# thawro/pytorch-human-pose

Hardware: AMD Instinct MI355X
Metric: images/sec (fwd+decode) HigherHRNet-W32 512px (higher is better)
Workload: dtype bf16; 1 GPU; HigherHRNet-W32 inference bf16, batch 32 @ 512x512 per GPU (conv fwd on N(0,1) images + AE decode on constructed maps, 10 people/image, det_thr 0.05, tag_thr 0.5, adjust+refine); global_batch=32, parallelism=image-sharded replicas x1, no data-path collective

## Files before the change

### include/hhrnet.h

```cpp
#ifndef HHRNET_H
#define HHRNET_H
#include <stdint.h>

#ifdef __cplusplus
extern "C" {
#endif

#define HH_ABI_VERSION 3
#define HH_DTYPE_BF16 1
#define HH_DTYPE_FP8 2
#define HH_DTYPE_F16 3

typedef struct hh_net hh_net;
typedef struct hh_decoder hh_decoder;

int hh_abi_version(void);
const char *hh_last_error(void);

hh_net *hh_create(int num_kpts, int C, int dtype);
void hh_destroy(hh_net *net);

hh_net *hh_create_classifier(int C, int num_classes, int dtype);
int hh_forward_classifier(hh_net *net, const float *images, int B, int H, int W, float *logits, void *stream);

int hh_num_params(const hh_net *net);
const char *hh_param_name(const hh_net *net, int index);
int hh_param_shape(const hh_net *net, int index, int64_t shape[4]);

int hh_load_weights(hh_net *net, const char *name, const float *host, const int64_t *shape, int ndim);
int hh_finalize(hh_net *net);

int hh_calibrate(hh_net *net, const float *images, int B, int H, int W, int rounds, void *stream);

int hh_e4m3_encode(const float *x, int64_t n, unsigned char *out);
int hh_e4m3_decode(const unsigned char *x, int64_t n, float *out);

int hh_reserve(hh_net *net, int B, int H, int W);
int64_t hh_workspace_bytes(const hh_net *net);

int hh_forward(hh_net *net, const float *images, int B, int H, int W, float *init_heatmaps, float *deconv_heatmaps,
               int use_graph, void *stream);

int hh_set_multi_lane(hh_net *net, int enable);

int hh_debug_check_plan(const hh_net *net);

double hh_forward_flops(const hh_net *net, int B, int H, int W);

int hh_profile_enable(hh_net *net, int enable);
int hh_profile_count(const hh_net *net);
int hh_profile_get(hh_net *net, int index, int *cfg, double *flops, double *bytes, float *ms, float *kernel_ms, const char **layer);
int hh_profile_clock(hh_net *net, int index, double *ghz);
int hh_conv_config(int cfg, int out[7]);
int hh_conv_config_double_buffered(int cfg);

int hh_debug_conv_bench(int cfg, int B, int Hin, int Win, int cin, int cout, int with_res, int relu, int iters,
                        float *ms_per_launch, unsigned long long *stamps16, int ref_cfg, float *max_diff);

int hh_debug_bb_bench(int B, int H, int W, int iters, float *ms_per_launch, unsigned long long *stamps64);
int hh_debug_bb_compare(int B, int H, int W, int iters, float *max_diff, float *ms_classic, float *ms_pc);

int hh_debug_bb_cover(int B, int H, int W, int tall, int num_cus, int64_t counts[4]);

int hh_debug_stem_fused(hh_net *net, const float *images, int B, int H, int W, void *out16, void *stream);

int hh_set_taps(hh_net *net, int enable);
int hh_num_taps(const hh_net *net);
const char *hh_tap_name(const hh_net *net, int index);
int hh_tap_shape(const hh_net *net, int index, int64_t shape[4]);
int hh_tap_read(hh_net *net, int index, float *host_nchw);

int hh_preprocess_u8(const unsigned char *image_hwc, int h, int w, const double dst_to_src[6], float *out_nchw, int H, int W,
                     const float mean[3], const float stdv[3], void *stream);

typedef struct hh_image_desc {
    long long offset;
    int h, w;
    double dst_to_src[6];
} hh_image_desc;
int hh_preprocess_u8_batch(const unsigned char *images_base, const hh_image_desc *descs_dev, int n, float *out_nchw, int H, int W,
                           const float mean[3], const float stdv[3], void *stream);

int hh_flip_images(const float *images, float *out, int B, int C, int H, int W, void *stream);
int hh_flip_merge(float *hm, int64_t hm_bstride, const float *hm_flipped, int64_t hmf_bstride, const float *tags_flipped,
                  int64_t tf_bstride, float *tags_out, int64_t to_bstride, const int32_t *perm_host, int B, int K,
                  int h, int w, void *stream);

hh_decoder *hh_decoder_create(int num_kpts, int max_people, double det_thr, double tag_thr);
void hh_decoder_destroy(hh_decoder *dec);
int hh_decoder_reserve(hh_decoder *dec, int B, int H, int W, int E);
int hh_decoder_set_exact_topk(hh_decoder *dec, int enable);

#define HH_DECODE_FALLBACK 1
#define HH_DECODE_SOLVER_GUARD 2
int hh_decode(hh_decoder *dec, const float *hm_q, int64_t hm_q_bstride, const float *hm_h, int64_t hm_h_bstride,
              const float *const *tags_q, const int64_t *tags_bstride, int E, int B, int hq, int wq, int adjust,
              int refine, float *joints, float *scores, int32_t *num_people, int32_t *flags, void *stream);

int hh_parse(hh_decoder *dec, const float *hm_full, const float *tags_full, int E, int B, int H, int W, int adjust,
             int refine, float *joints, float *scores, int32_t *num_people, int32_t *flags, void *stream);

int hh_loss_heatmaps(const float *pred, int64_t pred_bstride, const float *target, const float *mask, int B, int K, int h, int w,
                     float *loss, float *grad, int64_t grad_bstride, double *scratch, void *stream);
int hh_loss_ae_grouping(const float *tags, int64_t tags_bstride, const int32_t *joints, const int32_t *num_people, int B, int P, int K,
                        int h, int w, float *push_pull, float *grad, int64_t grad_bstride, float push_scale, float pull_scale,
                        double *scratch, void *stream);

#define HH_TRAIN_MAX_STAGES 4
typedef struct hh_train_desc {
    long long image_offset, mask_offset;
// ... 440 lines not shown
```

### pytorch-human-pose_amd/csrc/capi.cpp

```cpp
#include <algorithm>
#include <cmath>
#include <cstdint>
#include <cstring>
#include <string>
#include <vector>

#include "../../include/hhrnet.h"
#include "engine.h"
#include "optim_math.h"
#include "grad_stats_math.h"
#include "ema_math.h"
#include "render_math.h"
#include "text_math.h"
#include "seg_overlay_math.h"
#include "panel_math.h"
#include "coco_eval_math.h"
#include "pose_score_math.h"
#include "cls_score_math.h"
#include "crowd_mask_math.h"
#include "track_math.h"
#include "jpeg_math.h"
#include "jpeg_dec_math.h"

const char *hh_get_error();
int hh_tap_read_impl(hh_net *n, int index, float *host);

template <class Frame>
static int draw_check_frames(const char *fn, const hh_render_desc *descs_host, int n, const char *call_why, bool no_table, int th, int tw, int *max_tiles,
                             Frame frame)
{
    if (n <= 0 || n > 65535) { hh_set_error(std::string(fn) + ": need 0 < n <= 65535"); return 1; }
    if (call_why) { hh_set_error(std::string(fn) + ": " + call_why); return 1; }
    int tiles = 1;
    for (int b = 0; b < n; ++b) {
        const hh_render_desc &d = descs_host[b];
        if (d.prim_count > 0 && no_table) { hh_set_error(std::string(fn) + ": null primitive table"); return 1; }
        const char *why = frame(d);
        if (why) { hh_set_error(std::string(fn) + ": frame " + std::to_string(b) + ": " + why); return 1; }
        tiles = std::max(tiles, ((d.h + th - 1) / th) * ((d.w + tw - 1) / tw));
    }
    if (max_tiles) *max_tiles = tiles;
    return 0;
}

extern "C" {

int hh_abi_version(void) { return HH_ABI_VERSION; }
const char *hh_last_error(void) { return hh_get_error(); }

static bool f16_switch_refused(hh_net *n)
{
    if (n->dtype != HH_DTYPE_F16 || (!n->sw.no_stem_fused && !n->sw.bb32_tile)) return false;
    hh_set_error(std::string("hh_create: HH_DTYPE_F16 with ") + (n->sw.no_stem_fused ? "HH_NO_STEM_FUSED" : "HH_BB32=tile") +
                 ": that debug switch reaches a kernel that has no fp16 form");
    delete n;
    return true;
}

hh_net *hh_create(int num_kpts, int C, int dtype)
{
    if (dtype != HH_DTYPE_BF16 && dtype != HH_DTYPE_FP8 && dtype != HH_DTYPE_F16) {
// ... 2133 lines not shown
    double A[6][6] = {}, b[6];
    for (int i = 0; i < 3; ++i) {
        A[2 * i][0] = A[2 * i + 1][3] = from[i][0];
        A[2 * i][1] = A[2 * i + 1][4] = from[i][1];
        A[2 * i][2] = A[2 * i + 1][5] = 1;
        b[2 * i] = to[i][0];
        b[2 * i + 1] = to[i][1];
    }
    if (lu_solve6(A, b)) { hh_set_error("hh_get_affine_transform: degenerate point set (scale_w or dst_w is 0)"); return 1; }
    for (int i = 0; i < 6; ++i) out[i] = b[i];
    return 0;
}

int hh_invert_affine(const double m[6], double out[6])
{
#pragma clang fp contract(off)
    double M[6];
    for (int i = 0; i < 6; ++i) M[i] = m[i];
    double D = M[0] * M[4] - M[1] * M[3];
    D = D != 0 ? 1. / D : 0;
    const double A11 = M[4] * D, A22 = M[0] * D;
    M[0] = A11; M[1] *= -D;
    M[3] *= -D; M[4] = A22;
    const double b1 = -M[0] * M[2] - M[1] * M[5];
    const double b2 = -M[3] * M[2] - M[4] * M[5];
    M[2] = b1; M[5] = b2;
    for (int i = 0; i < 6; ++i) out[i] = M[i];
    return 0;
}

int hh_warp_affine_u8(const unsigned char *image_hwc, int h, int w, const double dst_to_src[6], unsigned char *out_hwc, int H, int W, void *stream)
{
    if (!image_hwc || !out_hwc || h <= 0 || w <= 0 || H <= 0 || W <= 0) { hh_set_error("hh_warp_affine_u8: bad argument"); return 1; }
    HH_CHECK_HIP(launch_warp_affine_u8(image_hwc, h, w, dst_to_src, out_hwc, H, W, (hipStream_t)stream));
    return 0;
}

int hh_transform_coords(const float *xy_in, int n, double cx, double cy, double scale_w, double dst_w, double dst_h,
                        double *xy_out)
{
#pragma clang fp contract(off)
    double M[6];
    if (hh_get_affine_transform(cx, cy, scale_w, dst_w, dst_h, 1, M)) return 1;
    for (int i = 0; i < n; ++i) {
        const double x = (double)xy_in[2 * i + 0], y = (double)xy_in[2 * i + 1];
        xy_out[2 * i + 0] = M[0] * x + M[1] * y + M[2] * 1.0;
        xy_out[2 * i + 1] = M[3] * x + M[4] * y + M[5] * 1.0;
    }
    return 0;
}

}

extern "C" int hh_debug_conv_bench(int cfg, int B, int Hin, int Win, int cin, int cout, int with_res, int relu, int iters,
                                   float *ms_per_launch, unsigned long long *stamps16, int ref_cfg, float *max_diff)
{
    HH_CHECK_HIP(conv_init());
    if (cfg < 0 || cfg >= conv_num_configs()) { hh_set_error("bad cfg"); return 1; }
    ConvConfig c = conv_config(cfg);
    if (cin % c.KC) { hh_set_error("cin must be a multiple of the config's KC"); return 1; }
    const int coutp = (cout + c.cout_t() - 1) / c.cout_t() * c.cout_t();
    const int Ho = c.S == 2 ? Hin / 2 : Hin, Wo = c.S == 2 ? Win / 2 : Win;
    const size_t n_in = (size_t)B * Hin * Win * cin, n_out = (size_t)B * Ho * Wo * coutp;
    std::vector<bf16_raw> h_in(n_in), h_res(n_out);
    std::vector<float> W((size_t)cout * cin * c.KS * c.KS), scale(coutp, 1.f);
    uint32_t s = 12345u;
    auto rnd = [&]() { s = s * 1664525u + 1013904223u; return (bf16_raw)(0x3c00u + ((s >> 16) & 0x1ffu) + ((s >> 30) << 15)); };
    auto rndf = [&]() { s = s * 1664525u + 1013904223u; return ((int)(s >> 20) - 2048) / 16384.0f; };
    for (auto &v : h_in) v = rnd();
    for (auto &v : h_res) v = rnd();
    for (auto &v : W) v = rndf();
    bf16_raw *d_in, *d_out, *d_out2, *d_res, *d_zero;
    float *d_bias;
    HH_CHECK_HIP(hipMalloc((void **)&d_in, n_in * 2));
    HH_CHECK_HIP(hipMalloc((void **)&d_out, n_out * 2));
    HH_CHECK_HIP(hipMalloc((void **)&d_out2, n_out * 2));
    HH_CHECK_HIP(hipMalloc((void **)&d_res, n_out * 2));
    HH_CHECK_HIP(hipMalloc((void **)&d_bias, (size_t)coutp * 4));
    HH_CHECK_HIP(hipMalloc((void **)&d_zero, 256));
    HH_CHECK_HIP(hipMemcpy(d_in, h_in.data(), n_in * 2, hipMemcpyHostToDevice));
    HH_CHECK_HIP(hipMemcpy(d_res, h_res.data(), n_out * 2, hipMemcpyHostToDevice));
    HH_CHECK_HIP(hipMemset(d_bias, 0, (size_t)coutp * 4));
    HH_CHECK_HIP(hipMemset(d_zero, 0, 256));
    HH_CHECK_HIP(hipMemset(d_out, 0, n_out * 2));
    HH_CHECK_HIP(hipMemset(d_out2, 0, n_out * 2));
    unsigned long long *d_st = nullptr;
    HH_CHECK_HIP(hipMalloc((void **)&d_st, 16 * 8));
    HH_CHECK_HIP(hipMemset(d_st, 0, 16 * 8));
    hipStream_t st;
    HH_CHECK_HIP(hipStreamCreate(&st));
    auto run = [&](int k, bf16_raw *out, int n, float *ms_out) -> int {
        const ConvConfig cc = conv_config(k);
        std::vector<bf16_raw> packed;
        hh_pack_weights(W.data(), scale.data(), cc.KS, cin, cout, cc.KC, cc.cout_t(), false, 0, 0, packed);
        bf16_raw *d_w;
        HH_CHECK_HIP(hipMalloc((void **)&d_w, packed.size() * 2));
        HH_CHECK_HIP(hipMemcpy(d_w, packed.data(), packed.size() * 2, hipMemcpyHostToDevice));
        ConvParams p{};
        p.in = d_in; p.in_cs = cin; p.Hin = Hin; p.Win = Win; p.w = d_w; p.bias = d_bias;
        p.res = with_res ? d_res : nullptr; p.res_cs = coutp;
        p.out = out; p.out_cs = coutp; p.Hob = Ho; p.Wob = Wo; p.osy = p.osx = 1;
        p.Ho = Ho; p.Wo = Wo; p.cin = cin; p.cout_real = cout; p.cout_store = coutp; p.relu = relu;
        p.pad_y = p.pad_x = (cc.KS - 1) / 2; p.B = B; p.stamps = d_st;
        p.tiles_x = (Wo + cc.TW - 1) / cc.TW; p.tiles_y = (Ho + cc.th() - 1) / cc.th(); p.ncg = coutp / cc.cout_t();
        auto launch = [&]() { return conv_launch(k, p, st); };
        hipEvent_t e0, e1;
        HH_CHECK_HIP(hipEventCreate(&e0));
        HH_CHECK_HIP(hipEventCreate(&e1));
        for (int i = 0; i < 3; ++i) HH_CHECK_HIP(launch());
        HH_CHECK_HIP(hipEventRecord(e0, st));
        for (int i = 0; i < n; ++i) HH_CHECK_HIP(launch());
        HH_CHECK_HIP(hipEventRecord(e1, st));
        HH_CHECK_HIP(hipEventSynchronize(e1));
        float ms = 0;
        HH_CHECK_HIP(hipEventElapsedTime(&ms, e0, e1));
        if (ms_out) *ms_out = ms / n;
        hipEventDestroy(e0); hipEventDestroy(e1); hipFree(d_w);
        return 0;
    };
    if (run(cfg, d_out, iters, ms_per_launch)) return 1;
    if (stamps16) HH_CHECK_HIP(hipMemcpy(stamps16, d_st, 16 * 8, hipMemcpyDeviceToHost));
    if (max_diff) {
        if (run(ref_cfg, d_out2, 1, nullptr)) return 1;
        std::vector<bf16_raw> a(n_out), b2(n_out);
        HH_CHECK_HIP(hipMemcpy(a.data(), d_out, n_out * 2, hipMemcpyDeviceToHost));
        HH_CHECK_HIP(hipMemcpy(b2.data(), d_out2, n_out * 2, hipMemcpyDeviceToHost));
        float md = 0.f;
        for (size_t i = 0; i < n_out; ++i) {
            uint32_t ua = (uint32_t)a[i] << 16, ub = (uint32_t)b2[i] << 16;
            float fa, fb;
            memcpy(&fa, &ua, 4); memcpy(&fb, &ub, 4);
            const float d = fa > fb ? fa - fb : fb - fa;
            if (d > md || d != d) md = d;
        }
        *max_diff = md;
    }
    hipStreamDestroy(st);
    hipFree(d_in); hipFree(d_out); hipFree(d_out2); hipFree(d_res); hipFree(d_bias); hipFree(d_st); hipFree(d_zero);
    return 0;
}

extern "C" int hh_debug_bb_cover(int B, int H, int W, int tall, int num_cus, int64_t counts[4])
{
    long long c[4];
    if (!counts) { hh_set_error("hh_debug_bb_cover: counts is NULL"); return 1; }
    if (!bbpc_cover(B, H, W, tall, num_cus, c)) { hh_set_error("hh_debug_bb_cover: the launcher does not take this shape"); return 1; }
    for (int i = 0; i < 4; ++i) counts[i] = c[i];
    return 0;
}

extern "C" int hh_debug_bb_compare(int B, int H, int W, int iters, float *max_diff, float *ms_classic, float *ms_pc)
{
    HH_CHECK_HIP(conv_init());
    HH_CHECK_HIP(bb_fused_init());
    HH_CHECK_HIP(bbpc_init());
    const size_t n = (size_t)B * H * W * 32;
    std::vector<bf16_raw> h_in(n), h_w(2 * 9 * 32 * 32), h_o1(n), h_o2(n);
    std::vector<float> h_b(64);
    uint32_t s = 4242u;
    auto rnd = [&]() { s = s * 1664525u + 1013904223u; return (bf16_raw)(0x3c00u + ((s >> 16) & 0x1ffu) + ((s >> 30) << 15)); };
    for (auto &v : h_in) v = (bf16_raw)(rnd() + 0x0300u);
    for (auto &v : h_w) v = rnd();
    for (auto &v : h_b) { s = s * 1664525u + 1013904223u; v = ((int)(s >> 20) - 2048) * 1e-4f; }
    bf16_raw *d_in, *d_o1, *d_o2, *d_w;
    float *d_b;
    HH_CHECK_HIP(hipMalloc((void **)&d_in, n * 2));
    HH_CHECK_HIP(hipMalloc((void **)&d_o1, n * 2));
    HH_CHECK_HIP(hipMalloc((void **)&d_o2, n * 2));
    HH_CHECK_HIP(hipMalloc((void **)&d_w, h_w.size() * 2));
    HH_CHECK_HIP(hipMalloc((void **)&d_b, 64 * 4));
    HH_CHECK_HIP(hipMemcpy(d_in, h_in.data(), n * 2, hipMemcpyHostToDevice));
    HH_CHECK_HIP(hipMemcpy(d_w, h_w.data(), h_w.size() * 2, hipMemcpyHostToDevice));
    HH_CHECK_HIP(hipMemcpy(d_b, h_b.data(), 64 * 4, hipMemcpyHostToDevice));
    HH_CHECK_HIP(hipMemset(d_o1, 0xff, n * 2));
    HH_CHECK_HIP(hipMemset(d_o2, 0xff, n * 2));
    BBParams p{};
    p.in = d_in; p.in_cs = 32; p.out_cs = 32; p.w1 = d_w; p.w2 = d_w + 9 * 32 * 32; p.b1 = d_b; p.b2 = d_b + 32;
    p.B = B; p.H = H; p.W = W;
    unsigned long long *d_st = nullptr;
    HH_CHECK_HIP(hipMalloc((void **)&d_st, 72 * 8));
    HH_CHECK_HIP(hipMemset(d_st, 0, 72 * 8));
    p.stamps = d_st;
    int dev = 0;
    hipDeviceProp_t prop;
    HH_CHECK_HIP(hipGetDevice(&dev));
    HH_CHECK_HIP(hipGetDeviceProperties(&prop, dev));
    hipStream_t st;
    HH_CHECK_HIP(hipStreamCreate(&st));
    hipEvent_t e0, e1;
    HH_CHECK_HIP(hipEventCreate(&e0));
    HH_CHECK_HIP(hipEventCreate(&e1));
// ... 95 lines not shown
```

### pytorch-human-pose_amd/csrc/engine.cpp

```cpp
#include "engine.h"
#include "f16_host.h"

#include <cmath>
#include <cstdlib>
#include <cstring>

static thread_local std::string g_err;
LaunchProbe &hh_launch_probe()
{
    static thread_local LaunchProbe p;
    return p;
}
void hh_set_error(const std::string &msg) { g_err = msg; }
const char *hh_get_error() { return g_err.c_str(); }

PlanSwitches PlanSwitches::from_env()
{
    auto on = [](const char *name) { const char *v = getenv(name); return v && *v && strcmp(v, "0"); };
    auto is = [](const char *name, const char *val) { const char *v = getenv(name); return v && !strcmp(v, val); };
    PlanSwitches s;
    s.bb32_tile = is("HH_BB32", "tile");
    s.no_bb64 = on("HH_NO_BB64");
    s.no_stem_fused = on("HH_NO_STEM_FUSED");
    s.no_junc_pair = on("HH_NO_JUNC_PAIR");
    s.full_join = on("HH_FULL_JOIN");
    s.no_fusion_merge = on("HH_NO_FUSION_MERGE");
    s.no_fused_upsum = on("HH_NO_FUSED_UPSUM");
    s.poison_ws = on("HH_POISON_WS");
    s.poison_lds = on("HH_POISON_LDS");
    s.no_head_fold = on("HH_NO_HEAD_FOLD");
    s.no_trans_dual = on("HH_NO_TRANS_DUAL");
    s.no_conv_db = on("HH_NO_CONV_DB");
    s.no_final_fuse = on("HH_NO_FINAL_FUSE");
    s.keep_waits = on("HH_KEEP_WAITS");
    s.event_system_fence = on("HH_EVENT_SYSTEM_FENCE");
    s.bb_tall = on("HH_NO_BB_TALL") ? 0 : is("HH_BB_TALL", "always") ? 2 : 1;
    s.fp8_trunk8 = is("HH_FP8_TRUNK", "e4m3");
    s.fp8_heads8 = is("HH_FP8_HEADS", "e4m3");
    return s;
}

static inline int round_up(int v, int m) { return (v + m - 1) / m * m; }

static inline bf16_raw f2bf(float f)
{
    uint32_t u;
    memcpy(&u, &f, 4);
    if ((u & 0x7fffffffu) > 0x7f800000u) return (bf16_raw)((u >> 16) | 0x40);
    u += 0x7fffu + ((u >> 16) & 1u);
    return (bf16_raw)(u >> 16);
}
static inline float bf2f(bf16_raw h)
{
    uint32_t u = (uint32_t)h << 16;
    float f;
    memcpy(&f, &u, 4);
    return f;
}
bf16_raw hh_net::cvt16(float f) const { return act() ? hh_f32_to_f16(f) : f2bf(f); }
float hh_net::widen16(bf16_raw v) const { return act() ? hh_f16_to_f32(v) : bf2f(v); }
int hh_net::check_packed(const std::vector<bf16_raw> &packed, const std::string &param_name) const
{
    if (!act()) return 0;
    for (bf16_raw v : packed)
        if (hh_f16_is_inf(v)) {
            hh_set_error("hh_finalize: " + param_name + ": a BatchNorm-folded weight exceeds the fp16 range (+-65504); use a bf16 handle for this checkpoint");
            return 1;
        }
    return 0;
}

int hh_net::add_param(const std::string &name, std::vector<int64_t> shape, bool counter)
{
    ParamSlot p;
    p.name = name;
    p.shape = std::move(shape);
    p.counter = counter;
    param_index[name] = (int)params.size();
    params.push_back(std::move(p));
    return (int)params.size() - 1;
}

namespace {
struct Builder {
// ... 506 lines not shown
                        for (int j = 0; j < 8; ++j, ++o) {
                            const int co = cg * COUT_T + ci_o, ci = ch * KC + c8 * 8 + j;
                            if (co >= cout || ci >= cin) continue;
                            float v;
                            if (transposed) v = W[(((size_t)ci * cout + co) * 4 + ky) * 4 + kx];
                            else v = W[(((size_t)co * cin + ci) * ks + ky) * ks + kx];
                            packed[o] = act_dtype ? hh_f32_to_f16(v * scale[co]) : f2bf(v * scale[co]);
                        }
            }
}

int hh_family_pick(int ks, int stride, int cin_pad, int coutp, int *KC, int *NT)
{
    if (ks == 3 && stride == 1) *KC = (cin_pad % 32 == 0) ? 32 : 16;
    else if (ks == 1) *KC = (cin_pad % 32 == 0) ? 32 : 16;
    else *KC = 16;
    *NT = (coutp % 64 == 0) ? 2 : 1;
    for (int i = 0; i < conv_num_configs(); ++i) {
        const ConvConfig &c = conv_config(i);
        if (c.KS == ks && c.S == stride && c.KC == *KC && c.NT == *NT && !c.DB) return 0;
    }
    return 1;
}

float hh_net::bn_fold(const std::string &bn, int co, const float *cb, float *shift) const
{
    const float g = param(bn + ".weight")[co], bta = param(bn + ".bias")[co];
    const float mu = param(bn + ".running_mean")[co], var = param(bn + ".running_var")[co];
    const float sc = g / std::sqrt(var + 1e-5f);
    *shift = cb ? bta + (*cb - mu) * sc : bta - mu * sc;
    return sc;
}

void hh_net::fold_layer(const ConvLayer &l, int coutp, std::vector<float> &scale, std::vector<float> &shift) const
{
    scale.assign(coutp, 0.f);
    shift.assign(coutp, 0.f);
    for (int co = 0; co < l.cout; ++co) {
        const float cb = l.bias.empty() ? 0.f : param(l.bias)[co];
        if (l.bn.empty()) { scale[co] = 1.f; shift[co] = cb; }
        else scale[co] = bn_fold(l.bn, co, &cb, &shift[co]);
    }
}

int hh_net::finalize()
{
    for (auto &p : params)
        if (!p.loaded && !p.counter) { hh_set_error("hh_finalize: parameter never loaded: " + p.name); return 1; }
    HH_CHECK_HIP(conv_init());
    HH_CHECK_HIP(bb_fused_init());
    HH_CHECK_HIP(stem_fused_init());
    HH_CHECK_HIP(bbpc_init());
    HH_CHECK_HIP(bb64_fused_init());
    HH_CHECK_HIP(junction_init());
    if (dtype == 2 && kind != 0) { hh_set_error("hh_finalize: the fp8 path covers HigherHRNet only"); return 1; }
    {
        int dev = 0;
        hipDeviceProp_t prop;
        HH_CHECK_HIP(hipGetDevice(&dev));
        HH_CHECK_HIP(hipGetDeviceProperties(&prop, dev));
        num_cus = prop.multiProcessorCount;
    }
    for (auto &l : layers) {
        if (l.stem) {
            const std::vector<float> &W = param(l.conv + ".weight");
            std::vector<bf16_raw> packed(64 * 32, 0);
            std::vector<float> shift(64);
            for (int co = 0; co < 64; ++co) {
                const float sc = bn_fold(l.bn, co, nullptr, &shift[co]);
                for (int t = 0; t < 27; ++t) {
                    const int kk = t / 16, hh = (t % 16) / 8, j = t % 8;
                    packed[((((co / 32) * 2 + kk) * 2 + hh) * 32 + co % 32) * 8 + j] = cvt16(W[(size_t)co * 27 + t] * sc);
                }
            }
            if (check_packed(packed, l.conv + ".weight")) return 1;
            if (hh_upload(&l.d_w, packed.data(), packed.size() * 2) || hh_upload(&l.d_bias, shift.data(), 64 * 4)) return 1;
            continue;
        }
        if (dtype == 2 && !l.hi) continue;
        const int cin_pad0 = round_up(l.cin, 16), coutp = round_up(l.cout, 32);
        if (l.stem2) { l.KC = 64; l.NT = 2; }
        else if (hh_family_pick(l.ks, l.stride, cin_pad0, coutp, &l.KC, &l.NT)) {
            hh_set_error("no kernel family for conv " + l.conv);
            return 1;
        }
        l.db = !sw.no_conv_db && !l.stem2 && l.ks == 3 && l.stride == 1 && !l.transposed && l.mconv.empty() && l.cin >= 128 &&
               l.cin % 16 == 0 && coutp % 64 == 0;
        if (l.db) { l.KC = 16; l.NT = 2; }
        l.cin_pad = round_up(l.cin, l.KC);
        const int COUT_T = 32 * l.NT;
        l.ncg = coutp / COUT_T;
        if (!l.mconv.empty()) {
            std::vector<float> Wm((size_t)l.cout * l.cin * 9, 0.f), one(coutp, 1.f), shift(coutp, 0.f);
            int c0 = 0;
            for (size_t m = 0; m < l.mconv.size(); ++m) {
                if (l.mcin[m] % l.KC) { hh_set_error("merged fusion conv: input width not a multiple of the chunk size"); return 1; }
                const std::vector<float> &Wj = param(l.mconv[m] + ".weight");
                for (int co = 0; co < l.cout; ++co) {
                    float sh;
                    const float sc = bn_fold(l.mbn[m], co, nullptr, &sh);
                    shift[co] += sh;
                    for (int ci = 0; ci < l.mcin[m]; ++ci)
                        for (int t = 0; t < 9; ++t) Wm[((size_t)co * l.cin + c0 + ci) * 9 + t] = Wj[((size_t)co * l.mcin[m] + ci) * 9 + t] * sc;
                    if (act())
                        for (int i = 0; i < l.mcin[m] * 9; ++i)
                            if (hh_f16_is_inf(hh_f32_to_f16(Wj[(size_t)co * l.mcin[m] * 9 + i] * sc))) return check_packed({0x7c00}, l.mconv[m] + ".weight");
// ... 418 lines not shown
    else if (act()) { hh_set_error("hh_forward: the tile-form 32-channel block (tensors of 2 GB and more) has no fp16 form"); return 1; }
    else HH_CHECK_HIP(bb_fused_launch(p, num_cus, s));
    return 0;
}

int hh_net::enqueue_conv(const Op &op, int B, int H, int W, float *o1, float *o2, hipStream_t s)
{
    const ConvLayer &l = layers[op.layer];
    const TensorDesc &ti = tensors[op.in];
    ConvParams p{};
    hh_conv_geometry(p, l, op, B, H >> ti.shift, W >> ti.shift, o1, o2);
    p.in = dtype == 2 ? ti.ptr16 : ti.ptr; p.in_cs = ti.C; p.in_coff = op.in_coff;
    p.w = l.d_w; p.bias = l.d_bias;
    if (op.out >= 0) {
        const TensorDesc &to = tensors[op.out];
        p.out = dtype == 2 ? to.ptr16 : to.ptr; p.out_cs = to.C; p.out_coff = op.out_coff;
    }
    if (op.res >= 0) {
        const TensorDesc &tr = tensors[op.res];
        p.res = dtype == 2 ? tr.ptr16 : tr.ptr; p.res_cs = tr.C; p.res_coff = op.res_coff;
    }
    if (op.in2 >= 0) {
        const TensorDesc &t2 = tensors[op.in2];
        if (t2.C != ti.C || t2.shift != ti.shift || (op.in3 >= 0 && (tensors[op.in3].C != ti.C || tensors[op.in3].shift != ti.shift))) {
            hh_set_error("merged fusion conv: inputs differ in shape or pixel stride");
            return 1;
        }
        p.nch0 = l.mcin[0] / l.KC;
        p.nch1 = l.mcin[1] / l.KC;
        p.src_delta1 = t2.ptr - (ti.ptr + op.in_coff);
        if (op.in3 >= 0) p.src_delta2 = tensors[op.in3].ptr - (ti.ptr + op.in_coff);
    }
    p.cout_store = op.cout_store >= 0 ? op.cout_store : round_up(l.cout, 8);
    if (op.layer2 >= 0) {
        const ConvLayer &l2 = layers[op.layer2];
        const TensorDesc &t2 = tensors[op.out2];
        const ConvConfig &c = conv_config(0);
        if (dtype == 2 || l.ks != 3 || l.stride != 1 || l.KC != c.KC || l.NT != c.NT || l.db || l.ncg != 1 || l2.ks != 3 || l2.stride != 2 || l2.KC != 16 ||
            l2.NT != 2 || l2.ncg != 1 || l2.cin_pad != l.cin_pad || t2.shift != ti.shift + 1) {
            hh_set_error("plan: the dual transition launch does not fit conv_mfma.hip (HH_NO_TRANS_DUAL=1)");
            return 1;
        }
        p.w2 = l2.d_w; p.bias2 = l2.d_bias;
        p.out2 = t2.ptr; p.out2_cs = t2.C; p.out2_coff = 0;
        p.Ho2 = p.Hin / 2; p.Wo2 = p.Win / 2;
        p.tiles_x = (p.Wo + c.TW - 1) / c.TW;
        p.tiles_y = (p.Ho + c.th() - 1) / c.th();
        if (prof_enabled && prof_record(op, HH_CFG_TRANS_DUAL, op_cost(op, B, H, W), &p.clk)) return 1;
        HH_CHECK_HIP(conv_dual_launch(p, s, act()));
        return 0;
    }
    const int cfg = hh_pick_config(l.ks, l.stride, l.KC, l.NT, p.Wo, l.db);
    const ConvConfig &c = conv_config(cfg);
    p.tiles_x = (p.Wo + c.TW - 1) / c.TW;
    p.tiles_y = (p.Ho + c.th() - 1) / c.th();
    if (prof_enabled && prof_record(op, cfg, op_cost(op, B, H, W), &p.clk)) return 1;
    HH_CHECK_HIP(conv_launch(cfg, p, s, act()));
    return 0;
}

int hh_net::forward(const float *images, int B, int H, int W, float *o1, float *o2, int use_graph, hipStream_t s)
{
    if (!finalized) { hh_set_error("hh_forward: call hh_finalize first"); return 1; }
    if (dtype == 2 && !calibrated) { hh_set_error("hh_forward: fp8 handle without activation scales, call hh_calibrate first"); return 1; }
    if (B > rB || H > rH || W > rW || !ws_ready || (taps_enabled && !taps.empty() && !taps[0].copy))
        if (reserve(B, H, W)) return 1;
    lastB = B; lastH = H; lastW = W;
    if (!use_graph || s == nullptr || taps_enabled || prof_enabled || sw.poison_lds || multi_lane)
        return enqueue(images, B, H, W, o1, o2, s);
    for (auto &g : graphs)
        if (g.images == images && g.o1 == o1 && g.o2 == o2 && g.B == B && g.H == H && g.W == W) {
            HH_CHECK_HIP(hipGraphLaunch(g.exec, s));
            return 0;
        }
    hipGraph_t graph;
    HH_CHECK_HIP(hipStreamBeginCapture(s, hipStreamCaptureModeThreadLocal));
    const int rc = enqueue(images, B, H, W, o1, o2, s);
    hipError_t e = hipStreamEndCapture(s, &graph);
    if (rc) return rc;
    HH_CHECK_HIP(e);
    GraphEntry g{images, o1, o2, B, H, W, nullptr};
    HH_CHECK_HIP(hipGraphInstantiate(&g.exec, graph, nullptr, nullptr, 0));
    hipGraphDestroy(graph);
    if (graphs.size() >= 8) {
        HH_CHECK_HIP(hipStreamSynchronize(s));
        hipGraphExecDestroy(graphs.front().exec);
        graphs.erase(graphs.begin());
    }
    graphs.push_back(g);
    HH_CHECK_HIP(hipGraphLaunch(g.exec, s));
    return 0;
}

int hh_net::check_plan(std::string *why) const
{
    struct Stamp { int lane; int t; int op; };
    LaneClocks lc;
    auto before = [&](const Stamp &st, int lane) { return st.lane < 0 || lc.behind(lane, st.lane, st.t); };
    std::vector<Stamp> writer(tensors.size(), Stamp{-1, 0, -1});
    std::vector<std::vector<Stamp>> readers(tensors.size());
    for (size_t i = 0; i < ops.size(); ++i) {
        const Op &op = ops[i];
        if (op.kind == OP_JOIN) { lc.join(op.nlanes); continue; }
        if (op.kind == OP_DEP) { lc.dep(op.lane, op.dep_from); continue; }
        if (op.kind == OP_MARK) { lc.set_mark(op.dep_from, op.nlanes); continue; }
        if (op.kind == OP_WAITL) {
// ... 176 lines not shown
```

### pytorch-human-pose_amd/csrc/engine.h

```cpp
#pragma once
#include <map>
#include <string>
#include <vector>

#include "kernels.h"

void hh_set_error(const std::string &msg);
void hh_pack_weights(const float *W, const float *scale, int ks, int cin, int cout, int KC, int COUT_T, bool transposed,
                     int py, int px, std::vector<unsigned short> &packed, int act_dtype = 0);
#define HH_CHECK_HIP(expr)                                                                             \
    do {                                                                                               \
        hipError_t _e = (expr);                                                                        \
        if (_e != hipSuccess) {                                                                        \
            hh_set_error(std::string(#expr) + ": " + hipGetErrorString(_e));                           \
            return 1;                                                                                  \
        }                                                                                              \
    } while (0)

struct ParamSlot {
    std::string name;
    std::vector<int64_t> shape;
    std::vector<float> data;
    bool loaded = false;
    bool counter = false;
// ... 50 lines not shown
    int scatter = 0;
    int up[3] = {-1, -1, -1}, up_shift[3] = {0, 0, 0}, nup = 0;
    int up_layer[3] = {-1, -1, -1};
    int C = 0;
    int tap = -1;
    bool res8 = false;
    int fin = -1;
    bool siblings = false;
    bool hi = false;
    int lane = 0;
    int nlanes = 0;
    int dep_from = 0;
    float s_in = 1.f, s_in2 = 1.f, s_res = 1.f, s_out = 1.f, s_up[3] = {1.f, 1.f, 1.f};
    float s_mid = 1.f;
    int amax_slot = -1;
};

struct TapInfo {
    std::string name;
    int tensor, coff, C;
    bf16_raw *copy = nullptr;
    float scale = 1.f;
    bool is16 = false;
};

struct ProfRecord {
    int op, cfg;
    double flops, bytes;
    hipEvent_t e0, e1;
    int slot;
};

struct GraphEntry {
    const void *images;
    void *o1, *o2;
    int B, H, W;
    hipGraphExec_t exec;
};

struct PlanSwitches {
    bool bb32_tile = false;
    bool no_bb64 = false;
    bool no_stem_fused = false;
    bool no_junc_pair = false;
    bool full_join = false;
    bool no_fusion_merge = false;
    bool no_fused_upsum = false;
    bool event_system_fence = false;
    bool keep_waits = false;
    bool no_final_fuse = false;
    int bb_tall = 1;
    bool no_conv_db = false;
    bool no_trans_dual = false;
    bool no_head_fold = false;
    bool fp8_trunk8 = false;
    bool fp8_heads8 = false;
    bool poison_ws = false;
    bool poison_lds = false;
    static PlanSwitches from_env();
};

struct OpCost { double flops = 0, bytes = 0; };

struct hh_net {
    int K, C, dtype;
    int kind = 0;
    int num_classes = 0;
    float *d_pool = nullptr, *d_fc_w = nullptr, *d_fc_b = nullptr;
    int pool_cap = 0;
    std::vector<ParamSlot> params;
    std::map<std::string, int> param_index;
    std::vector<ConvLayer> layers;
    std::vector<TensorDesc> tensors;
    std::vector<Op> ops;
    std::vector<TapInfo> taps;
    bool taps_enabled = false;
    bool finalized = false;
    int num_cus = 256;
    int rB = 0, rH = 0, rW = 0;
    int lastB = 0, lastH = 0, lastW = 0;
    int64_t ws_bytes = 0;
    bool ws_ready = false;
    std::vector<void *> allocs;
    std::vector<GraphEntry> graphs;
    bool prof_enabled = false;
    bool prof_clk = false;
    std::vector<ProfRecord> prof;
    size_t prof_used = 0;
    unsigned long long *d_clk = nullptr;
    double clk_khz = 0;
    hipStream_t lane_streams[4] = {nullptr, nullptr, nullptr, nullptr};
    int lane_priority = 0;
    bool lane_priority_set = false;
    std::vector<hipEvent_t> lane_events;
    size_t lane_events_used = 0;
    bool multi_lane = true;
    PlanSwitches sw;
    bool calibrated = false;
    bool calibrating = false;
    unsigned *d_amax = nullptr;
    std::vector<float> amax;
    int elem() const { return dtype == 2 ? 1 : 2; }
    bool is16() const { return dtype != 2; }
    int act() const { return dtype == 3 ? 1 : 0; }
    bf16_raw cvt16(float f) const;
    float widen16(bf16_raw v) const;
// ... 67 lines not shown
```

### pytorch-human-pose_amd/csrc/kernels.h

```cpp
#pragma once
#include <hip/hip_runtime.h>
#include <stdint.h>

#include <hip/hip_ext.h>

#include "../../include/hhrnet.h"

typedef uint16_t bf16_raw;

struct LaunchProbe { hipEvent_t start = nullptr, stop = nullptr; };
LaunchProbe &hh_launch_probe();
#define HH_LAUNCH(kernel, grid, block, lds, stream, ...)                                                            \
    do {                                                                                                            \
        LaunchProbe &lp_ = hh_launch_probe();                                                                       \
        if (lp_.start) {                                                                                            \
            hipExtLaunchKernelGGL(kernel, grid, block, lds, stream, lp_.start, lp_.stop, 0, __VA_ARGS__);           \
            lp_ = LaunchProbe{};                                                                                    \
        } else {                                                                                                    \
            hipLaunchKernelGGL(kernel, grid, block, lds, stream, __VA_ARGS__);                                      \
        }                                                                                                           \
    } while (0)

struct ConvParams {
    const bf16_raw *in;
    int in_cs, in_coff;
    int Hin, Win;
    const bf16_raw *w;
    const float *bias;
    const bf16_raw *res;
    int res_cs, res_coff;
    bf16_raw *out;
    int out_cs, out_coff;
    float *out_f32;
    int Hob, Wob;
    int osy, ooy, osx, oox;
    int Ho, Wo;
    int cin;
    int cout_real, cout_store;
    int relu;
    int pad_y, pad_x;
    int B, tiles_x, tiles_y, ncg;
    int nphase;
    size_t phase_stride;
    unsigned long long *stamps;
    unsigned long long *clk;
    int nch0, nch1;
    ptrdiff_t src_delta1, src_delta2;
    const bf16_raw *w2;
    const float *bias2;
    bf16_raw *out2;
    int out2_cs, out2_coff;
    int Ho2, Wo2;
};

struct ConvConfig {
    int KS, S, KC, NT, WC, PT, TW;
    int DB;
    int cout_t() const { return 32 * NT * WC; }
    int th() const { return (4 / WC) * PT * (32 / TW); }
    size_t lds_bytes() const {
        int PH = (th() - 1) * S + KS, PW = (TW - 1) * S + KS;
        size_t patch = ((size_t)PH * PW * (KC * 2 + 16) + 15) & ~(size_t)15;
        const size_t buf = patch + (size_t)KS * KS * KC * cout_t() * 2;
        return DB ? 2 * (buf + 256 * 16) : buf;
    }
};

int conv_num_configs();
const ConvConfig &conv_config(int i);
hipError_t conv_launch(int cfg_index, const ConvParams &p, hipStream_t stream, int act_dtype = 0);
hipError_t conv_init();
#define HH_CFG_TRANS_DUAL 108
hipError_t conv_dual_launch(const ConvParams &p, hipStream_t stream, int act_dtype = 0);

struct Fp8ConvParams {
    const unsigned char *in;
    int in_cs, in_coff;
    int Hin, Win;
    const unsigned char *w;
    const float *mult;
    const float *bias;
    const unsigned char *res;
    int res_cs, res_coff;
    float res_scale;
    const bf16_raw *res16;
    int res16_cs, res16_coff;
    unsigned char *out;
    int out_cs, out_coff;
    float out_inv_scale;
    bf16_raw *out16;
    int out16_cs, out16_coff;
    float *out_f32;
    int Hob, Wob;
    int osy, ooy, osx, oox;
    int Ho, Wo;
    int cin;
    int cout_real, cout_store;
    int relu;
    int pad_y, pad_x;
    int B, tiles_x, tiles_y, ncg;
    int nphase;
    size_t phase_stride;
    unsigned *absmax;
};
struct Fp8ConvConfig {
    int KS, S, KC, NT, PT, TW;
    static constexpr int pixel_stride(int kc) { return ((kc / 16 + 1) | 1) * 16; }
    int cout_t() const { return 32 * NT; }
    int th() const { return 4 * PT * (32 / TW); }
    int nstep() const { return (KS * KS * (KC / 16) + 3) / 4; }
    size_t lds_bytes() const {
        const int PH = (th() - 1) * S + KS, PW = (TW - 1) * S + KS;
        const size_t patch = ((size_t)PH * PW * pixel_stride(KC) + 15) & ~(size_t)15;
        return patch + (size_t)nstep() * 4 * cout_t() * 16;
    }
};
int conv_fp8_num_configs();
const Fp8ConvConfig &conv_fp8_config(int i);
hipError_t conv_fp8_launch(int cfg_index, const Fp8ConvParams &p, hipStream_t stream);
hipError_t conv_fp8_init();

struct Fp8BBParams {
    const unsigned char *in; int in_cs;
    unsigned char *out; int out_cs;
    const unsigned char *w1, *w2;
    const float *mult1, *bias1, *mult2, *bias2;
// ... 302 lines not shown
```

Measured before the change: 6934 images/sec.

## Add persistent weight-stationary kernel for 64->64 3x3 convs

Adds a persistent conv kernel for 3x3 stride-1 64->64 channel convolutions without residual. Each workgroup keeps all weights in registers and loops over spatial tiles with a grid capped at the CU count. The next tile's input patch is prefetched into a double-buffered LDS area while MFMAs run, with explicit scheduling barriers to interleave them. It is selected by default for 16-bit activations when there are at least twice as many tiles as CUs. The cost is heavy register use (one workgroup per CU) and possible load imbalance on the last tiles.

Result: no change. 6977 images/sec, median of 6 (+0.6%).

```diff
diff --git a/include/hhrnet.h b/include/hhrnet.h
--- a/include/hhrnet.h
+++ b/include/hhrnet.h
@@ -56,6 +56,10 @@
 
 int hh_debug_conv_bench(int cfg, int B, int Hin, int Win, int cin, int cout, int with_res, int relu, int iters,
                         float *ms_per_launch, unsigned long long *stamps16, int ref_cfg, float *max_diff);
+#define HH_CFG_CONV64_WS 109
+int hh_debug_conv_bench_elem(int act_dtype, int cfg, int B, int Hin, int Win, int cin, int cout, int with_res, int relu, int iters,
+                           float *ms_per_launch, unsigned long long *stamps16, int ref_cfg, float *max_diff);
+int hh_debug_conv64_cover(int B, int H, int W, int num_wgs, int64_t counts[2]);
 
 int hh_debug_bb_bench(int B, int H, int W, int iters, float *ms_per_launch, unsigned long long *stamps64);
 int hh_debug_bb_compare(int B, int H, int W, int iters, float *max_diff, float *ms_classic, float *ms_pc);
diff --git a/pytorch-human-pose_amd/csrc/capi.cpp b/pytorch-human-pose_amd/csrc/capi.cpp
--- a/pytorch-human-pose_amd/csrc/capi.cpp
+++ b/pytorch-human-pose_amd/csrc/capi.cpp
@@ -7,6 +7,7 @@
 
 #include "../../include/hhrnet.h"
 #include "engine.h"
+#include "f16_host.h"
 #include "optim_math.h"
 #include "grad_stats_math.h"
 #include "ema_math.h"
@@ -2246,11 +2247,29 @@
 
 }
 
-extern "C" int hh_debug_conv_bench(int cfg, int B, int Hin, int Win, int cin, int cout, int with_res, int relu, int iters,
-                                   float *ms_per_launch, unsigned long long *stamps16, int ref_cfg, float *max_diff)
+static int conv_bench(int act_dtype, int cfg, int B, int Hin, int Win, int cin, int cout, int with_res, int relu, int iters,
+                      float *ms_per_launch, unsigned long long *stamps16, int ref_cfg, float *max_diff)
 {
     HH_CHECK_HIP(conv_init());
-    if (cfg < 0 || cfg >= conv_num_configs()) { hh_set_error("bad cfg"); return 1; }
+    if (act_dtype != 0 && act_dtype != 1) { hh_set_error("hh_debug_conv_bench: act_dtype is 0 (bf16) or 1 (fp16)"); return 1; }
+    const bool ws = cfg == HH_CFG_CONV64_WS;
+    if (ws) {
+        if (cin != 64 || cout != 64 || with_res) { hh_set_error("hh_debug_conv_bench: the weight-stationary conv is 64 -> 64 channels without residual"); return 1; }
+        HH_CHECK_HIP(conv64_ws_init());
+        cfg = 1;
+        const ConvConfig &c1 = conv_config(1);
+        if (c1.KS != 3 || c1.S != 1 || c1.KC != 32 || c1.NT != 2 || c1.WC != 1) { hh_set_error("hh_debug_conv_bench: config 1 is not the 64-cout 3x3 form"); return 1; }
+    }
+    if (cfg < 0 || cfg >= conv_num_configs() || (max_diff && (ref_cfg < 0 || ref_cfg >= conv_num_configs()))) { hh_set_error("bad cfg"); return 1; }
+    if (B <= 0 || Hin <= 0 || Win <= 0 || cin <= 0 || cout <= 0 || iters <= 0) { hh_set_error("hh_debug_conv_bench: empty shape"); return 1; }
+    int num_cus = 0;
+    {
+        int dev = 0;
+        HH_CHECK_HIP(hipGetDevice(&dev));
+        HH_CHECK_HIP(hipDeviceGetAttribute(&num_cus, hipDeviceAttributeMultiprocessorCount, dev));
+    }
+    const char *pz = getenv("HH_POISON_LDS");
+    const bool poison = pz && *pz && strcmp(pz, "0");
     ConvConfig c = conv_config(cfg);
     if (cin % c.KC) { hh_set_error("cin must be a multiple of the config's KC"); return 1; }
     const int coutp = (cout + c.cout_t() - 1) / c.cout_t() * c.cout_t();
@@ -2283,10 +2302,10 @@
     HH_CHECK_HIP(hipMemset(d_st, 0, 16 * 8));
     hipStream_t st;
     HH_CHECK_HIP(hipStreamCreate(&st));
-    auto run = [&](int k, bf16_raw *out, int n, float *ms_out) -> int {
+    auto run = [&](int k, bool use_ws, bf16_raw *out, int n, float *ms_out) -> int {
         const ConvConfig cc = conv_config(k);
         std::vector<bf16_raw> packed;
-        hh_pack_weights(W.data(), scale.data(), cc.KS, cin, cout, cc.KC, cc.cout_t(), false, 0, 0, packed);
+        hh_pack_weights(W.data(), scale.data(), cc.KS, cin, cout, cc.KC, cc.cout_t(), false, 0, 0, packed, act_dtype);
         bf16_raw *d_w;
         HH_CHECK_HIP(hipMalloc((void **)&d_w, packed.size() * 2));
         HH_CHECK_HIP(hipMemcpy(d_w, packed.data(), packed.size() * 2, hipMemcpyHostToDevice));
@@ -2297,7 +2316,10 @@
         p.Ho = Ho; p.Wo = Wo; p.cin = cin; p.cout_real = cout; p.cout_store = coutp; p.relu = relu;
         p.pad_y = p.pad_x = (cc.KS - 1) / 2; p.B = B; p.stamps = d_st;
         p.tiles_x = (Wo + cc.TW - 1) / cc.TW; p.tiles_y = (Ho + cc.th() - 1) / cc.th(); p.ncg = coutp / cc.cout_t();
-        auto launch = [&]() { return conv_launch(k, p, st); };
+        auto launch = [&]() {
+            if (poison) { const hipError_t e = launch_lds_poison(num_cus, st); if (e != hipSuccess) return e; }
+            return use_ws ? conv64_ws_launch(p, num_cus, st, act_dtype) : conv_launch(k, p, st, act_dtype);
+        };
         hipEvent_t e0, e1;
         HH_CHECK_HIP(hipEventCreate(&e0));
         HH_CHECK_HIP(hipEventCreate(&e1));
@@ -2312,10 +2334,10 @@
         hipEventDestroy(e0); hipEventDestroy(e1); hipFree(d_w);
         return 0;
     };
-    if (run(cfg, d_out, iters, ms_per_launch)) return 1;
+    if (run(cfg, ws, d_out, iters, ms_per_launch)) return 1;
     if (stamps16) HH_CHECK_HIP(hipMemcpy(stamps16, d_st, 16 * 8, hipMemcpyDeviceToHost));
     if (max_diff) {
-        if (run(ref_cfg, d_out2, 1, nullptr)) return 1;
+        if (run(ref_cfg, false, d_out2, 1, nullptr)) return 1;
         std::vector<bf16_raw> a(n_out), b2(n_out);
         HH_CHECK_HIP(hipMemcpy(a.data(), d_out, n_out * 2, hipMemcpyDeviceToHost));
         HH_CHECK_HIP(hipMemcpy(b2.data(), d_out2, n_out * 2, hipMemcpyDeviceToHost));
@@ -2324,6 +2346,7 @@
             uint32_t ua = (uint32_t)a[i] << 16, ub = (uint32_t)b2[i] << 16;
             float fa, fb;
             memcpy(&fa, &ua, 4); memcpy(&fb, &ub, 4);
+            if (act_dtype) { fa = hh_f16_to_f32(a[i]); fb = hh_f16_to_f32(b2[i]); }
             const float d = fa > fb ? fa - fb : fb - fa;
             if (d > md || d != d) md = d;
         }
@@ -2331,6 +2354,25 @@
     }
     hipStreamDestroy(st);
     hipFree(d_in); hipFree(d_out); hipFree(d_out2); hipFree(d_res); hipFree(d_bias); hipFree(d_st); hipFree(d_zero);
+    return 0;
+}
+extern "C" int hh_debug_conv_bench(int cfg, int B, int Hin, int Win, int cin, int cout, int with_res, int relu, int iters,
+                                   float *ms_per_launch, unsigned long long *stamps16, int ref_cfg, float *max_diff)
+{
+    return conv_bench(0, cfg, B, Hin, Win, cin, cout, with_res, relu, iters, ms_per_launch, stamps16, ref_cfg, max_diff);
+}
+extern "C" int hh_debug_conv_bench_elem(int act_dtype, int cfg, int B, int Hin, int Win, int cin, int cout, int with_res, int relu, int iters,
+                                      float *ms_per_launch, unsigned long long *stamps16, int ref_cfg, float *max_diff)
+{
+    return conv_bench(act_dtype, cfg, B, Hin, Win, cin, cout, with_res, relu, iters, ms_per_launch, stamps16, ref_cfg, max_diff);
+}
+
+extern "C" int hh_debug_conv64_cover(int B, int H, int W, int num_wgs, int64_t counts[2])
+{
+    long long c[2];
+    if (!counts) { hh_set_error("hh_debug_conv64_cover: counts is NULL"); return 1; }
+    if (!conv64_cover(B, H, W, num_wgs, c)) { hh_set_error("hh_debug_conv64_cover: empty shape, no workgroups, or 2^31 pixels and more"); return 1; }
+    counts[0] = c[0]; counts[1] = c[1];
     return 0;
 }
 
diff --git a/pytorch-human-pose_amd/csrc/conv64_ws.hip b/pytorch-human-pose_amd/csrc/conv64_ws.hip
--- /dev/null
+++ b/pytorch-human-pose_amd/csrc/conv64_ws.hip
@@ -0,0 +1,226 @@
+#include "mfma_dev.h"
+
+#include <stdlib.h>
+
+namespace {
+constexpr int TH = CONV64_TH, TW = CONV64_TW;
+constexpr int PH = TH + 2, PW = TW + 2;
+constexpr int PS = 64 * 2 + 16;
+constexpr int NTHR = 512;
+constexpr int PPIX = PH * PW;
+constexpr int NPL = (PPIX * 8 + NTHR - 1) / NTHR;
+constexpr int BUF_BYTES = NPL * NTHR / 8 * PS;
+constexpr int WCH = 9 * 4 * 64;
+constexpr int NSTEP = 2 * 6 * 4;
+}
+
+size_t conv64_ws_lds_bytes() { return 2 * BUF_BYTES + 64 * 4; }
+
+template <typename E>
+__global__ __launch_bounds__(NTHR, 1) void conv64_ws_kernel(const ConvParams p)
+{
+    extern __shared__ __attribute__((aligned(16))) char smem[];
+    float *lds_b = reinterpret_cast<float *>(smem + 2 * BUF_BYTES);
+
+    const int tid = threadIdx.x;
+    if (p.clk && tid == 0) atomicMin(p.clk, wall_clock64());
+    const int wave = tid >> 6, lane = tid & 63;
+    const int r = lane & 31, h = lane >> 5;
+    const int ct = wave & 1, part = wave >> 1;
+    const int ntiles = p.B * p.tiles_y * p.tiles_x, tiles_per_img = p.tiles_y * p.tiles_x;
+
+    u32x4 wa[36];
+    {
+        const u32x4 *wl = reinterpret_cast<const u32x4 *>(p.w) + h * 64 + ct * 32 + r;
+        static_for<36>([&](auto jc) {
+            constexpr int j = decltype(jc)::value, c = j / 18, kx = (j % 18) / 6, kk = (j % 6) / 3, ky = j % 3;
+            wa[j] = wl[c * WCH + ((ky * 3 + kx) * 4 + kk * 2) * 64];
+        });
+    }
+
+    int pl_yx[NPL];
+#pragma unroll
+    for (int i = 0; i < NPL; ++i) {
+        const int u = tid + NTHR * i, pix = (u >> 7) * 16 + (u & 15);
+        pl_yx[i] = pix < PPIX ? (((pix / PW) << 8) | (pix % PW)) : -1;
+    }
+    const int prt8 = ((tid >> 4) & 7) * 8;
+    const int wbase = ((tid >> 7) * 16 + (tid & 15)) * PS + ((tid >> 4) & 7) * 16;
+    const int bbase = (part * 2 * PW + r) * PS + h * 16;
+
+    u32x4 preg[NPL];
+    const bf16_raw *pf_base = p.in;
+    int pf_iy0 = 0, pf_ix0 = 0;
+    bool pf_more = true;
+    auto pf_setup = [&](int ti) {
+        const Conv64Geom g = conv64_geom(conv64_band(ti, ntiles, gridDim.x), p.tiles_x, tiles_per_img);
+        pf_iy0 = g.oy0 - 1; pf_ix0 = g.ox0 - 1;
+        pf_base = p.in + p.in_coff + (((ptrdiff_t)g.b * p.Hin + pf_iy0) * p.Win + pf_ix0) * p.in_cs;
+    };
+    auto pf_load = [&](auto ic) {
+        constexpr int i = decltype(ic)::value;
+        const int py = pl_yx[i] >> 8, px = pl_yx[i] & 255;
+        const bool ok = pf_more & (pl_yx[i] >= 0) & ((unsigned)(pf_iy0 + py) < (unsigned)p.Hin) & ((unsigned)(pf_ix0 + px) < (unsigned)p.Win);
+        preg[i] = *reinterpret_cast<const u32x4 *>(ok ? pf_base + (py * p.Win + px) * p.in_cs + prt8 : p.zeros);
+    };
+    auto write_unit = [&](auto ic, int boff) {
+        constexpr int i = decltype(ic)::value;
+        *reinterpret_cast<u32x4 *>(smem + boff + wbase + i * (NTHR / 8 * PS)) = preg[i];
+    };
+
+    int t = blockIdx.x;
+    pf_setup(t);
+    static_for<NPL>(pf_load);
+    if (tid < 64) lds_b[tid] = p.bias[tid];
+    static_for<NPL>([&](auto ic) { write_unit(ic, 0); });
+    __syncthreads();
+
+    const short fl = p.relu ? (short)0 : (short)-32768;
+    const i16x2 floor = {fl, fl};
+    int roff = 0;
+    for (; t < ntiles; t += gridDim.x) {
+        const Conv64Geom g = conv64_geom(conv64_band(t, ntiles, gridDim.x), p.tiles_x, tiles_per_img);
+        const int tn = t + gridDim.x;
+        pf_more = tn < ntiles;
+        pf_setup(pf_more ? tn : t);
+        const int woff = BUF_BYTES - roff;
+
+        f32x16 acc[2];
+#pragma unroll
+        for (int q = 0; q < 4; ++q) {
+            const float4 bv = *reinterpret_cast<const float4 *>(lds_b + ct * 32 + 8 * q + 4 * h);
+#pragma unroll
+            for (int pt = 0; pt < 2; ++pt) {
+                acc[pt][4 * q + 0] = bv.x + 0.f; acc[pt][4 * q + 1] = bv.y + 0.f; acc[pt][4 * q + 2] = bv.z + 0.f; acc[pt][4 * q + 3] = bv.w + 0.f;
+            }
+        }
+        __builtin_amdgcn_sched_barrier(0);
+
+        const char *lds_r = smem + roff + bbase;
+        u32x4 fb[3];
+        auto ldb = [&](int s, int buf) {
+            const int cb = s >> 2, i = s & 3, c = cb / 6, kx = (cb % 6) >> 1, kk = cb & 1;
+            fb[buf] = *reinterpret_cast<const u32x4 *>(lds_r + (i * PW + kx) * PS + c * 64 + kk * 32);
+        };
+        ldb(0, 0);
+        ldb(1, 1);
+        __builtin_amdgcn_sched_group_barrier(0x100, 2, 0);
+        static_for<NSTEP>([&](auto sc) {
+            constexpr int s = decltype(sc)::value, cb = s >> 2, i = s & 3;
+            if constexpr (s + 2 < NSTEP) {
+                ldb(s + 2, (s + 2) % 3);
+                __builtin_amdgcn_sched_group_barrier(0x100, 1, 0);
+            }
+            if constexpr (s < NPL) {
+                pf_load(sc);
+                __builtin_amdgcn_sched_group_barrier(0x020, 1, 0);
+            }
+            if constexpr (s >= NSTEP - NPL) {
+                write_unit(std::integral_constant<int, s - (NSTEP - NPL)>{}, woff);
+                __builtin_amdgcn_sched_group_barrier(0x200, 1, 0);
+            }
+            constexpr int nm = (i == 0 || i == 3) ? 1 : 2;
+            static_for<3>([&](auto kyc) {
+                constexpr int ky = decltype(kyc)::value, pt = i - ky;
+                if constexpr (pt >= 0 && pt < 2) acc[pt] = E::mfma(wa[cb * 3 + ky], fb[s % 3], acc[pt]);
+            });
+            __builtin_amdgcn_sched_group_barrier(0x8, nm, 0);
+        });
+
+#pragma unroll
+        for (int pt = 0; pt < 2; ++pt) {
+            const int oy = g.oy0 + part * 2 + pt, ox = g.ox0 + r;
+            const bool valid = oy < p.Ho && ox < p.Wo;
+            const size_t pix = ((size_t)g.b * p.Ho + oy) * p.Wo + ox;
+#pragma unroll
+            for (int m = 0; m < 2; ++m) {
+                const unsigned x0 = E::pack(acc[pt][8 * m + 0], acc[pt][8 * m + 1], floor);
+                const unsigned x1 = E::pack(acc[pt][8 * m + 2], acc[pt][8 * m + 3], floor);
+                const unsigned y0 = E::pack(acc[pt][8 * m + 4], acc[pt][8 * m + 5], floor);
+                const unsigned y1 = E::pack(acc[pt][8 * m + 6], acc[pt][8 * m + 7], floor);
+                auto s0 = __builtin_amdgcn_permlane32_swap(x0, y0, false, false);
+                auto s1 = __builtin_amdgcn_permlane32_swap(x1, y1, false, false);
+                if (valid) *reinterpret_cast<u32x4 *>(p.out + pix * p.out_cs + p.out_coff + ct * 32 + 16 * m + 8 * h) = u32x4{s0[0], s1[0], s0[1], s1[1]};
+            }
+        }
+        lds_barrier();
+        roff = woff;
+    }
+    if (p.clk && tid == 0) atomicMax(p.clk + 1, wall_clock64());
+}
+
+bool conv64_ws_supported(const ConvParams &p)
+{
+    return p.in && p.w && p.bias && p.out && !p.res && !p.out_f32 && !p.w2 && p.cin == 64 && p.cout_real == 64 && p.cout_store == 64 && p.ncg == 1 &&
+           p.nphase <= 1 && p.nch0 == 0 && p.pad_y == 1 && p.pad_x == 1 && p.osy == 1 && p.osx == 1 && p.ooy == 0 && p.oox == 0 && p.Ho == p.Hin &&
+           p.Wo == p.Win && p.Hob == p.Ho && p.Wob == p.Wo && p.B > 0 && p.Hin > 0 && p.Win > 0 && p.in_cs % 8 == 0 && p.in_coff % 8 == 0 &&
+           p.out_cs % 8 == 0 && p.out_coff % 8 == 0 && p.in_cs >= 64 && p.out_cs >= 64 &&
+           (long long)p.Hin * p.Win * p.in_cs < (1ll << 31) &&
+           (long long)p.B * ((p.Hin + TH - 1) / TH) * ((p.Win + TW - 1) / TW) < (1ll << 30);
+}
+
+static bf16_raw *g_conv64_zeros[64] = {};
+
+hipError_t conv64_ws_init()
+{
+    int dev = 0;
+    hipError_t e = hipGetDevice(&dev);
+    if (e != hipSuccess) return e;
+    if (!g_conv64_zeros[dev & 63]) {
+        bf16_raw *z = nullptr;
+        e = hipMalloc((void **)&z, 256);
+        if (e != hipSuccess) return e;
+        e = hipMemset(z, 0, 256);
+        if (e != hipSuccess) { (void)hipFree(z); return e; }
+        g_conv64_zeros[dev & 63] = z;
+    }
+    e = hipFuncSetAttribute(reinterpret_cast<const void *>(conv64_ws_kernel<ElemBF16>), hipFuncAttributeMaxDynamicSharedMemorySize,
+                                       (int)conv64_ws_lds_bytes());
+    if (e != hipSuccess) return e;
+    return hipFuncSetAttribute(reinterpret_cast<const void *>(conv64_ws_kernel<ElemF16>), hipFuncAttributeMaxDynamicSharedMemorySize,
+                               (int)conv64_ws_lds_bytes());
+}
+
+hipError_t conv64_ws_launch(ConvParams p, int num_cus, hipStream_t s, int act_dtype)
+{
+    if ((act_dtype != 0 && act_dtype != 1) || num_cus <= 0 || !conv64_ws_supported(p)) return hipErrorInvalidValue;
+    int dev = 0;
+    if (hipGetDevice(&dev) != hipSuccess || !g_conv64_zeros[dev & 63]) return hipErrorNotInitialized;
+    p.zeros = g_conv64_zeros[dev & 63];
+    p.tiles_x = (p.Wo + TW - 1) / TW;
+    p.tiles_y = (p.Ho + TH - 1) / TH;
+    if (const char *v = getenv("HH_CONV64_WS_GRID")) {
+        const int cap = atoi(v);
+        if (cap > 0 && cap < num_cus) num_cus = cap;
+    }
+    const int grid = conv64_grid(p.B * p.tiles_y * p.tiles_x, num_cus);
+    if (act_dtype) HH_LAUNCH(conv64_ws_kernel<ElemF16>, dim3(grid), dim3(NTHR), conv64_ws_lds_bytes(), s, p);
+    else HH_LAUNCH(conv64_ws_kernel<ElemBF16>, dim3(grid), dim3(NTHR), conv64_ws_lds_bytes(), s, p);
+    return hipGetLastError();
+}
+
+bool conv64_cover(int B, int H, int W, int num_wgs, long long counts[2])
+{
+    if (B <= 0 || H <= 0 || W <= 0 || num_wgs <= 0 || (long long)B * H * W >= (1ll << 31)) return false;
+    const int tiles_x = (W + TW - 1) / TW, tiles_y = (H + TH - 1) / TH, tiles_per_img = tiles_x * tiles_y, ntiles = B * tiles_per_img;
+    const int grid = conv64_grid(ntiles, num_wgs);
+    unsigned char *n = (unsigned char *)calloc((size_t)B * H * W, 1);
+    if (!n) return false;
+    for (int wg = 0; wg < grid; ++wg)
+        for (int t = wg; t < ntiles; t += grid) {
+            const Conv64Geom g = conv64_geom(conv64_band(t, ntiles, (unsigned)grid), tiles_x, tiles_per_img);
+            for (int wv = 0; wv < NTHR / 64; ++wv)
+                for (int pt = 0; pt < 2; ++pt)
+                    for (int r = 0; r < 32; ++r) {
+                        const int oy = g.oy0 + (wv >> 1) * 2 + pt, ox = g.ox0 + r;
+                        if ((wv & 1) == 0 && g.b < B && oy < H && ox < W) {
+                            unsigned char &c = n[((size_t)g.b * H + oy) * W + ox];
+                            if (c < 255) ++c;
+                        }
+                    }
+        }
+    counts[0] = counts[1] = 0;
+    for (size_t i = 0; i < (size_t)B * H * W; ++i) { counts[0] += n[i] == 0; counts[1] += n[i] > 1; }
+    free(n);
+    return true;
+}
diff --git a/pytorch-human-pose_amd/csrc/engine.cpp b/pytorch-human-pose_amd/csrc/engine.cpp
--- a/pytorch-human-pose_amd/csrc/engine.cpp
+++ b/pytorch-human-pose_amd/csrc/engine.cpp
@@ -30,6 +30,7 @@
     s.poison_lds = on("HH_POISON_LDS");
     s.no_head_fold = on("HH_NO_HEAD_FOLD");
     s.no_trans_dual = on("HH_NO_TRANS_DUAL");
+    s.conv64_ws = on("HH_NO_CONV64_WS") ? 0 : is("HH_CONV64_WS", "always") ? 2 : 1;
     s.no_conv_db = on("HH_NO_CONV_DB");
     s.no_final_fuse = on("HH_NO_FINAL_FUSE");
     s.keep_waits = on("HH_KEEP_WAITS");
@@ -642,6 +643,7 @@
     HH_CHECK_HIP(stem_fused_init());
     HH_CHECK_HIP(bbpc_init());
     HH_CHECK_HIP(bb64_fused_init());
+    HH_CHECK_HIP(conv64_ws_init());
     HH_CHECK_HIP(junction_init());
     if (dtype == 2 && kind != 0) { hh_set_error("hh_finalize: the fp8 path covers HigherHRNet only"); return 1; }
     {
@@ -1166,6 +1168,13 @@
     }
     const int cfg = hh_pick_config(l.ks, l.stride, l.KC, l.NT, p.Wo, l.db);
     const ConvConfig &c = conv_config(cfg);
+    const int ws_tiles = B * ((p.Ho + CONV64_TH - 1) / CONV64_TH) * ((p.Wo + CONV64_TW - 1) / CONV64_TW);
+    if (is16() && sw.conv64_ws && (sw.conv64_ws == 2 || ws_tiles >= 2 * num_cus) && l.ks == 3 && l.stride == 1 && !l.transposed && l.cin == 64 && l.cout == 64 && l.KC == 32 && l.NT == 2 &&
+        c.TW == 32 && c.PT == 2 && c.WC == 1 && !c.DB && op.in2 < 0 && conv64_ws_supported(p)) {
+        if (prof_enabled && prof_record(op, HH_CFG_CONV64_WS, op_cost(op, B, H, W), &p.clk)) return 1;
+        HH_CHECK_HIP(conv64_ws_launch(p, num_cus, s, act()));
+        return 0;
+    }
     p.tiles_x = (p.Wo + c.TW - 1) / c.TW;
     p.tiles_y = (p.Ho + c.th() - 1) / c.th();
     if (prof_enabled && prof_record(op, cfg, op_cost(op, B, H, W), &p.clk)) return 1;
diff --git a/pytorch-human-pose_amd/csrc/engine.h b/pytorch-human-pose_amd/csrc/engine.h
--- a/pytorch-human-pose_amd/csrc/engine.h
+++ b/pytorch-human-pose_amd/csrc/engine.h
@@ -126,6 +126,7 @@
     int bb_tall = 1;
     bool no_conv_db = false;
     bool no_trans_dual = false;
+    int conv64_ws = 1;
     bool no_head_fold = false;
     bool fp8_trunk8 = false;
     bool fp8_heads8 = false;
diff --git a/pytorch-human-pose_amd/csrc/kernels.h b/pytorch-human-pose_amd/csrc/kernels.h
--- a/pytorch-human-pose_amd/csrc/kernels.h
+++ b/pytorch-human-pose_amd/csrc/kernels.h
@@ -51,6 +51,7 @@
     bf16_raw *out2;
     int out2_cs, out2_coff;
     int Ho2, Wo2;
+    const bf16_raw *zeros;
 };
 
 struct ConvConfig {
@@ -72,6 +73,24 @@
 hipError_t conv_init();
 #define HH_CFG_TRANS_DUAL 108
 hipError_t conv_dual_launch(const ConvParams &p, hipStream_t stream, int act_dtype = 0);
+
+constexpr int CONV64_TH = 8, CONV64_TW = 32;
+struct Conv64Geom { int b, oy0, ox0; };
+__host__ __device__ inline int conv64_grid(int ntiles, int num_cus) { return ntiles < num_cus ? ntiles : num_cus; }
+__host__ __device__ inline int conv64_band(int i, int ntiles, unsigned grid)
+{
+    return ((ntiles & 7) == 0 && (grid & 7) == 0) ? (i & 7) * (ntiles >> 3) + (i >> 3) : i;
+}
+__host__ __device__ inline Conv64Geom conv64_geom(int tile, int tiles_x, int tiles_per_img)
+{
+    const int b = tile / tiles_per_img, tt = tile % tiles_per_img;
+    return Conv64Geom{b, (tt / tiles_x) * CONV64_TH, (tt % tiles_x) * CONV64_TW};
+}
+size_t conv64_ws_lds_bytes();
+hipError_t conv64_ws_init();
+bool conv64_ws_supported(const ConvParams &p);
+hipError_t conv64_ws_launch(ConvParams p, int num_cus, hipStream_t s, int act_dtype = 0);
+bool conv64_cover(int B, int H, int W, int num_wgs, long long counts[2]);
 
 struct Fp8ConvParams {
     const unsigned char *in;
```
